# Avielstein/GRASP_LAB_SALP

Measured on AMD Instinct MI355X. Metric: env-steps/sec at 65536 parallel envs, 1/2/4/8 MI355X; % HBM roofline, higher is better.
Workload: dtype f64

## Files before the change

### grasp_lab_salp_amd/csrc/salp_device.h

```cpp
#ifndef SALP_DEVICE_H
#define SALP_DEVICE_H

#include <hip/hip_runtime.h>
#include <stdint.h>

#include "../../include/salp.h"
#include "salp_math.h"
#include "salp_philox.h"
#include "salp_random.h"

#pragma clang fp contract(off)

static_assert(SALP_FMA, "libsalp.so is built in the product arithmetic mode (salp_math.h)");

#define SD static __device__ __forceinline__
#define SD_MEMBER __device__ __forceinline__
#define SD_HOST_DEV static __host__ __device__ __forceinline__

namespace salp {

constexpr double DT = 0.01;
constexpr double PI = 3.141592653589793;
constexpr double COS_GAMMA = 0x1.6a09e667f3bcdp-1;
constexpr double SIN_GAMMA = 0x1.6a09e667f3bccp-1;
// ... 69 lines not shown
    if (d != 0.0 && fabs(d) * 2.0 == fabs(ulp) && e != 0.0) r = ((e > 0) == (d > 0)) ? nb : r;
    return r;
}

struct Rot { double r[3][3]; };
SD Rot rot_sc(double sp, double cp, double st, double ct, double ss, double cs) {
    double a00 = cs * ct, a01 = -ss, a02 = cs * st;
    double a10 = ss * ct, a11 = cs, a12 = ss * st;
    double a20 = -st, a22 = ct;
    Rot R;
    R.r[0][0] = a00; R.r[0][1] = sm_fma(a02, sp, a01 * cp); R.r[0][2] = sm_fma(a02, cp, a01 * -sp);
    R.r[1][0] = a10; R.r[1][1] = sm_fma(a12, sp, a11 * cp); R.r[1][2] = sm_fma(a12, cp, a11 * -sp);
    R.r[2][0] = a20; R.r[2][1] = a22 * sp;                   R.r[2][2] = a22 * cp;
    return R;
}
SD Rot rot_zyx(double phi, double theta, double psi) {
    double sp, cp, st, ct, ss, cs;
    sm_sincos(phi, &sp, &cp);
    sm_sincos(theta, &st, &ct);
    sm_sincos(psi, &ss, &cs);
    return rot_sc(sp, cp, st, ct, ss, cs);
}
SD void world_frame(double e0, double e1, double e2, double v0, double v1, double v2, double* o, SmPoly K) {
    double sp, cp, st, ct, ss, cs;
    sm_sincos_rp2(e0, e1, &sp, &cp, &st, &ct, K);
    sm_sincos_yaw_p(e2, &ss, &cs, K);
    sm_world_frame(sp, cp, st, ct, ss, cs, v0, v1, v2, o);
}
SD void rot_body_xy(const Rot& R, double d0, double d1, double* b0, double* b1) {
    *b0 = sm_fma(R.r[1][0], d1, R.r[0][0] * d0);
    *b1 = sm_fma(R.r[1][1], d1, R.r[0][1] * d0);
}

SD double r32(double x, bool f) { return f ? (double)(float)x : x; }
SD double sel(bool f, double c) { return f ? (double)(float)c : c; }
// ... 319 lines not shown
    SF(SALP_F_POS0) = h.q0; SF(SALP_F_POS1) = h.q1; SF(SALP_F_POS2) = h.q2;
    SF(SALP_F_ANG0) = h.g0; SF(SALP_F_ANG1) = h.g1; SF(SALP_F_ANG2) = h.g2;
    SF(SALP_F_LENGTH) = h.L; SF(SALP_F_WIDTH) = h.W; SF(SALP_F_VOLUME) = h.V;
    SF(SALP_F_PREV_VOLUME) = h.pV; SF(SALP_F_COM) = h.com; SF(SALP_F_COM_RATE) = h.comr;
    SF(SALP_F_COM_ACC) = h.coma;
    SF(SALP_F_PREV_I0) = h.pI0; SF(SALP_F_PREV_I1) = h.pI1; SF(SALP_F_PREV_I2) = h.pI2;
    SF(SALP_F_GEOM32) = h.g32 ? 1.0 : 0.0; SF(SALP_F_PVOL32) = h.pv32 ? 1.0 : 0.0;
    SF(SALP_F_CYCLE_TIME) = h.ct; SF(SALP_F_TIME) = h.time;
    SF(SALP_F_REFILL_TIME) = h.refill; SF(SALP_F_JET_TIME) = h.jet; SF(SALP_F_COAST_TIME) = h.coast;
    SF(SALP_F_CONTRACTION) = h.c; SF(SALP_F_CONTRACT_RATE) = h.cr; SF(SALP_F_RELEASE_RATE) = h.rr;
    SF(SALP_F_TURN_TIME) = h.turn;
    SF(SALP_F_PHASE) = (double)h.phase;
    SF(SALP_F_CONTR32) = h.c32 ? 1.0 : 0.0;
}

SD void nozzle_direction(double angle1, double angle2, double* d) {
    const double cg = COS_GAMMA, sg = SIN_GAMMA;
    double s1, c1, s2, c2;
    sm_sincos(angle1, &s1, &c1);
    sm_sincos(angle2, &s2, &c2);
    double n00 = cg * c2, n10 = s2, n20 = sg * c2;
    double n02 = -sg, n12 = 0.0, n22 = cg;
    double c00 = -n20, c02 = -n22;
    double c10 = sm_fma(c1, n10, s1 * n00), c12 = sm_fma(c1, n12, s1 * n02);
    double c20 = sm_fma(-s1, n10, c1 * n00), c22 = sm_fma(-s1, n12, c1 * n02);
    d[0] = sm_fma(c02, sg, c00 * cg);
    d[1] = sm_fma(c12, sg, c10 * cg);
    d[2] = sm_fma(c22, sg, c20 * cg);
}
SD void cycle_bounds(Hot& h) {
    h.mx = pymax(h.refill, h.turn);
    h.b1 = h.mx + h.jet;
    h.b2 = h.b1 + h.coast;
}

// ... 208 lines not shown
        ng.m = k32[C32_M]; ng.I0 = k32[C32_I0]; ng.I1 = k32[C32_I1];
        ng.kc0 = k32[C32_KC0]; ng.kc1 = k32[C32_KC1]; ng.ra0 = k32[C32_RA0]; ng.ra1 = k32[C32_RA1];
        ng.dimx = k32[C32_DIMX]; ng.dimy = k32[C32_DIMY];
    }
    h.V = V;
    double comr = div_dt(com - h.com);
    h.coma = div_dt(comr - h.comr);
    h.com = com;
    h.comr = comr;
    jet_rates(P, V, h.pV, wm, f, h.pv32, ng);
    geo_recips(ng);
    h.geo = ng;
    return false;
}

SD void nozzle_ik(double yaw, bool yaw32, double* an1_out, double* an2_out) {
    double sy, cy;
    if (yaw32) {
        float s, c;
        sm_np_sincosf((float)yaw, &s, &c);
        sy = s; cy = c;
    } else {
        sm_sincos(yaw, &sy, &cy);
    }
    double t1 = -sy, t2 = cy;
    double val2 = 2.0 * t2 - 1.0;
    if (val2 < -1.0) val2 = -1.0;
    if (val2 > 1.0) val2 = 1.0;
    double an2 = sm_acos(val2), an1;
    if (an2 <= -PI) an2 += 2 * PI;
    else if (an2 > PI) an2 -= 2 * PI;
    if (an2 == 0.0) {
        an1 = 0.0;
    } else {
        double s2, c2;
        sm_sincos(an2, &s2, &c2);
        double a = 0.5 * (c2 - 1.0);
        double b = sqrt(2.0) * s2 / 2.0;
        double val1 = t1 / sqrt(a * a + b * b);
        if (val1 < -1.0) val1 = -1.0;
        if (val1 > 1.0) val1 = 1.0;
        an1 = sm_asin(val1) - sm_atan2(b, a);
    }
    if (an1 <= -PI) an1 += 2 * PI;
    else if (an1 > PI) an1 -= 2 * PI;
    *an1_out = an1;
    *an2_out = an2;
}
template <class ST>
SD void nozzle_solve(ST S, const Params& P, int64_t i, double yaw, bool yaw32) {
    SF(SALP_F_PREV_YAW) = SF(SALP_F_YAW);
    SF(SALP_F_YAW) = yaw;
    SF(SALP_F_PREV_ANGLE1) = SF(SALP_F_ANGLE1);
    SF(SALP_F_PREV_ANGLE2) = SF(SALP_F_ANGLE2);
    double an1, an2;
    nozzle_ik(yaw, yaw32, &an1, &an2);
    SF(SALP_F_ANGLE1) = an1;
    SF(SALP_F_ANGLE2) = an2;
}

SD int predict_cycle_ticks(const Params& P, float a0, float a1, float a2, double* ang1, double* ang2) {
    const float r0 = a0 * 0.06f, r1 = a1 * 10.0f, r2 = a2 * (float)(PI / 2);
    double an1, an2;
    nozzle_ik((double)r2, true, &an1, &an2);
    const double turn = fabs(an1 - *ang1) / P.angle_speed + fabs(an2 - *ang2) / P.angle_speed;
    *ang1 = an1;
    *ang2 = an2;
    const double c = (double)r0, sq = (double)sqf(r0);
    const double refill = REFILL_C0 * sq + REFILL_C1 * c + REFILL_C2;
    const double jet = PROPUL_C0 * sq + PROPUL_C1 * c + PROPUL_C2;
    const double total = pymax(refill, turn) + jet + (double)r1;
// ... 22 lines not shown
    } else {
        sr_coef_means(&k);
    }
    SF(SALP_F_CD) = k.cd; SF(SALP_F_DFR) = k.dfr; SF(SALP_F_DTR) = k.dtr;
#pragma unroll
    for (int j = 0; j < 3; ++j) {
        SF(SALP_F_AMF0 + j) = k.amf[j]; SF(SALP_F_AMRF0 + j) = k.amrf[j];
        SF(SALP_F_AMT0 + j) = k.amt[j]; SF(SALP_F_AMRT0 + j) = k.amrt[j];
    }
    h.rnd.cd = k.cd; h.rnd.dfr = k.dfr; h.rnd.dtr = k.dtr;
    h.rnd.amf0 = k.amf[0]; h.rnd.amf1 = k.amf[1]; h.rnd.amf2 = k.amf[2];
    h.rnd.amrf0 = k.amrf[0]; h.rnd.amrf1 = k.amrf[1]; h.rnd.amrf2 = k.amrf[2];
    h.rnd.amt0 = k.amt[0]; h.rnd.amt1 = k.amt[1]; h.rnd.amt2 = k.amt[2];
}

template <bool RAND = false, class ST>
SD void set_control(Hot& h, ST S, const Params& P, int64_t i, double contraction, double coast,
                    double a1, double a2, bool c32) {
    set_coefficients<RAND>(h, S, P, i);
    SF(SALP_F_AVGV0) = 0.0; SF(SALP_F_AVGV1) = 0.0; SF(SALP_F_AVGV2) = 0.0;
    SF(SALP_F_AVGW0) = 0.0; SF(SALP_F_AVGW1) = 0.0; SF(SALP_F_AVGW2) = 0.0;
    h.c = contraction;
    h.coast = coast;
    h.c32 = c32;
    h.turn = nozzle_set_angles(S, P, i, a1, a2);
    nozzle_direction(a1, a2, &h.d0);
    SF(SALP_F_CYCLE) = SF(SALP_F_CYCLE) + 1.0;
    h.ct = 0.0;
    const double sq = c32 ? (double)sqf((float)h.c) : h.c * h.c;
    h.refill = REFILL_C0 * sq + REFILL_C1 * h.c + REFILL_C2;
    h.jet = PROPUL_C0 * sq + PROPUL_C1 * h.c + PROPUL_C2;
    h.cr = h.refill > 0 ? h.c / h.refill : 0.0;
    h.rr = h.jet > 0 ? h.c / h.jet : 0.0;
    cycle_bounds(h);
}

template <class ST>
SD void cycle_prologue(const Hot& h, ST S, const Params& P, int64_t i) {
    const double total = h.b2;
    double pq0 = SF(SALP_F_PPOS0), pq1 = SF(SALP_F_PPOS1), pq2 = SF(SALP_F_PPOS2);
    double pg0 = SF(SALP_F_PANG0), pg1 = SF(SALP_F_PANG1), pg2 = SF(SALP_F_PANG2);
    SF(SALP_F_AVGV0) = (h.q0 - pq0) / total; SF(SALP_F_AVGV1) = (h.q1 - pq1) / total;
    SF(SALP_F_AVGV2) = (h.q2 - pq2) / total;
    SF(SALP_F_AVGW0) = (h.g0 - pg0) / total; SF(SALP_F_AVGW1) = (h.g1 - pg1) / total;
    SF(SALP_F_AVGW2) = (h.g2 - pg2) / total;
    SF(SALP_F_PPOS0) = h.q0; SF(SALP_F_PPOS1) = h.q1; SF(SALP_F_PPOS2) = h.q2;
    SF(SALP_F_PANG0) = h.g0; SF(SALP_F_PANG1) = h.g1; SF(SALP_F_PANG2) = h.g2;
    SF(SALP_F_PENDING) = 1.0;
}

template <bool RAND = false, class ST>
SD void begin_step(Hot& h, ST S, const Params& P, int64_t i, float a0, float a1, float a2,
                   Cache32 c32) {
    SF(SALP_F_ACT0) = a0; SF(SALP_F_ACT1) = a1; SF(SALP_F_ACT2) = a2;
    float r0 = a0 * 0.06f, r1 = a1 * 10.0f, r2 = a2 * (float)(PI / 2);
    if (RAND && P.rand_act) {
        const float rr[3] = {r0, r1, r2};
        double ra[3];
        sr_randomize_action(P.seed, h.env_id, (uint64_t)SF(SALP_F_STEP_COUNT), rr, ra);
        nozzle_solve(S, P, i, ra[2], false);
        set_control<RAND>(h, S, P, i, ra[0], ra[1], SF(SALP_F_ANGLE1), SF(SALP_F_ANGLE2), false);
    } else {
        nozzle_solve(S, P, i, (double)r2, true);
        set_control<RAND>(h, S, P, i, (double)r0, (double)r1, SF(SALP_F_ANGLE1), SF(SALP_F_ANGLE2), true);
    }
    fill_cache32(P, h.c, c32);
    cycle_prologue(h, S, P, i);
}

template <class ST>
SD void record_state(const Hot& h, const Params& P, ST S, int64_t i, double* rec,
                     int64_t rs, bool first) {
    auto put = [&](int col, double x) { rec[(int64_t)col * rs] = x; };
    put(SALP_T_STATE, (double)h.phase);
    put(SALP_T_PW0, h.p0); put(SALP_T_PW1, h.p1); put(SALP_T_PW2, h.p2);
    put(SALP_T_V0, h.v0); put(SALP_T_V1, h.v1); put(SALP_T_V2, h.v2);
    put(SALP_T_ACC0, h.a0); put(SALP_T_ACC1, h.a1); put(SALP_T_ACC2, h.a2);
    put(SALP_T_ETA0, h.e0); put(SALP_T_ETA1, h.e1); put(SALP_T_ETA2, h.e2);
    put(SALP_T_W0, h.w0); put(SALP_T_W1, h.w1); put(SALP_T_W2, h.w2);
// ... 16 lines not shown
        for (int k = SALP_T_FIRST_FORCE; k < SALP_TRACE_DIM; ++k) put(k, NAN);
        put(SALP_T_ETAR0, NAN); put(SALP_T_ETAR1, NAN); put(SALP_T_ETAR2, NAN);
        put(SALP_T_NOZZLE_YAW, NAN);
    } else {
        const double yaw = SF(SALP_F_YAW), pyaw = SF(SALP_F_PREV_YAW);
        put(SALP_T_NOZZLE_YAW, h.ct < h.turn ? pyaw + (h.ct / h.turn) * (yaw - pyaw) : yaw);
    }
}

template <class ST>
SD void resume_cycle(Hot& h, ST S, const Params& P, int64_t i) {
    cycle_bounds(h);
    nozzle_direction(SF(SALP_F_ANGLE1), SF(SALP_F_ANGLE2), &h.d0);
}

template <class ST>
SD void observation(const Hot& h, const Rot& R, ST S, const Params& P, int64_t i,
                    float* obs) {
    double tx = SF(SALP_F_TARGET0), ty = SF(SALP_F_TARGET1);
    double b0, b1;
    rot_body_xy(R, tx - h.p0, ty - h.p1, &b0, &b1);
    double heading = sm_atan2(b1, b0);
    obs[0] = (float)b0; obs[1] = (float)b1;
    obs[2] = (float)h.v0; obs[3] = (float)h.v1;
    obs[4] = (float)h.w2; obs[5] = (float)heading;
    const int nob = (int)SF(SALP_F_N_OBST);
#pragma unroll
    for (int k = 0; k < SALP_MAX_OBSTACLES; ++k) {
        if (k >= P.num_obstacles) break;
        if (k < nob) {
            obs[6 + 2 * k] = (float)(SF(SALP_F_OBST0 + 2 * k) - h.p0);
            obs[7 + 2 * k] = (float)(SF(SALP_F_OBST0 + 2 * k + 1) - h.p1);
        } else {
            obs[6 + 2 * k] = 0.0f;
            obs[7 + 2 * k] = 0.0f;
        }
    }
}

struct StepOut {
    double reward;
    bool terminated, truncated, hit;
};

template <bool RAND = false, class ST>
SD StepOut finish_step(Hot& h, ST S, const Params& P, int64_t i, float* obs,
                       double* info) {
    StepOut out;
    const Rot R = rot_zyx(h.e0, h.e1, h.e2);
    double vw[3];
    world_frame(h.e0, h.e1, h.e2, h.v0, h.v1, h.v2, vw, sm_poly());
    const double px = h.p0, py = h.p1;
    double path = SF(SALP_F_PATH_LEN) + np_norm2(px - SF(SALP_F_LAST_PX), py - SF(SALP_F_LAST_PY));
    SF(SALP_F_PATH_LEN) = path;
    SF(SALP_F_LAST_PX) = px; SF(SALP_F_LAST_PY) = py;
    double svel = SF(SALP_F_SUM_VEL) + np_norm2(vw[0], vw[1]);
    SF(SALP_F_SUM_VEL) = svel;
    const double tx = SF(SALP_F_TARGET0), ty = SF(SALP_F_TARGET1);
    const double dx = px - tx, dy = py - ty;
    const double dist = np_norm2(dx, dy);
    double comp[7];
    comp[0] = (-dist + SF(SALP_F_PREV_DIST)) * 100;
    SF(SALP_F_PREV_DIST) = dist;
    double b0, b1;
    rot_body_xy(R, dx, dy, &b0, &b1);
    comp[1] = -0.5 * fabs(sm_atan2(-b1, -b0));
    const float a2 = (float)SF(SALP_F_ACT2);
    const double ep_len = SF(SALP_F_EP_LEN);
    if (ep_len == 0.0) {
        double ch = (double)a2 - SF(SALP_F_PREV_A2);
        comp[2] = -1.0 * (ch * ch);
    } else {
        float ch = a2 - (float)SF(SALP_F_PREV_A2);
        comp[2] = (double)(-(ch * ch));
    }
    comp[3] = -10.0 * fabs(SF(SALP_F_AVGW2));
    comp[4] = -0.1;
    comp[5] = -100.0 * fabs(SF(SALP_F_AVGV1));
    comp[6] = 0.0;
    const int nob = (int)SF(SALP_F_N_OBST);
    double md = 0.0;
#pragma unroll
    for (int k = 0; k < SALP_MAX_OBSTACLES; ++k) {
        if (k >= nob) break;
        double d = np_norm2(px - SF(SALP_F_OBST0 + 2 * k), py - SF(SALP_F_OBST0 + 2 * k + 1));
        if (k == 0 || d < md) md = d;
    }
    if (nob > 0) {
        double danger = 2.0 * P.obstacle_radius;
        if (md < danger) comp[6] = -1.0 * (1.0 - md / danger);
    }
    double reward = comp[0] + comp[1] + comp[2] + comp[3] + comp[4] + comp[5] + comp[6];
    observation(h, R, S, P, i, obs);
    if (RAND && P.rand_obs) sr_randomize_obs(P.seed, h.env_id, (uint64_t)SF(SALP_F_STEP_COUNT), obs);
    bool l32;
    double Lc, Wc;
    body_lw(P, h.phase, h.ct, h.refill, h.mx, h.c, h.cr, h.rr, h.c32, &Lc, &Wc, &l32);
    double thr = l32 ? (double)((float)P.obstacle_radius + (float)Lc / 2.0f)
                     : P.obstacle_radius + Lc / 2;
    bool hit = false;
#pragma unroll
    for (int k = 0; k < SALP_MAX_OBSTACLES; ++k) {
        if (k >= nob) break;
        double d = np_norm2(px - SF(SALP_F_OBST0 + 2 * k), py - SF(SALP_F_OBST0 + 2 * k + 1));
        if (d < thr) hit = true;
    }
    bool done = false, trunc = false;
    if (dist < 0.2) { done = true; reward += 500.0; }
    else if (dist > 5.0) { trunc = true; reward -= 200.0; }
    if (hit) { trunc = true; reward -= 200.0; }
    if (SF(SALP_F_CYCLE) >= (double)P.max_cycles) { trunc = true; reward -= 50.0; }
    const double nlen = ep_len + 1.0;
    SF(SALP_F_EP_LEN) = nlen;
    const double ret = SF(SALP_F_EP_RETURN) + reward;
    SF(SALP_F_EP_RETURN) = ret;
    const double sa0 = SF(SALP_F_SUM_A0) + (double)(float)SF(SALP_F_ACT0);
    const double sa1 = SF(SALP_F_SUM_A1) + (double)(float)SF(SALP_F_ACT1);
    const double sa2 = SF(SALP_F_SUM_ABS_A2) + (double)fabsf(a2);
    SF(SALP_F_SUM_A0) = sa0; SF(SALP_F_SUM_A1) = sa1; SF(SALP_F_SUM_ABS_A2) = sa2;
// ... 16 lines not shown
            info[SALP_INFO_DIRECT_DISTANCE] = dd;
            info[SALP_INFO_PATH_EFFICIENCY] = path > 0 ? dd / path : 0.0;
            info[SALP_INFO_FINAL_DISTANCE] = dist;
            info[SALP_INFO_INITIAL_DISTANCE] = SF(SALP_F_INIT_DIST);
            info[SALP_INFO_AVG_COMPRESSION] = sa0 / nlen;
            info[SALP_INFO_AVG_COAST_TIME] = sa1 / nlen;
            info[SALP_INFO_AVG_NOZZLE_ANGLE] = sa2 / nlen;
            info[SALP_INFO_AVG_VELOCITY] = svel / (nlen + 1.0);
            for (int k = 0; k < 7; ++k) info[SALP_INFO_AVG_R_TRACK + k] = sr[k] / nlen;
        }
    }
    SF(SALP_F_PREV_A2) = (double)a2;
    SF(SALP_F_PENDING) = 0.0;
    if (RAND && P.latency) {
        const double lat = sr_latency(P.seed, h.env_id, (uint64_t)SF(SALP_F_STEP_COUNT));
        set_control<RAND>(h, S, P, i, 0.0, lat, SF(SALP_F_ANGLE1), SF(SALP_F_ANGLE2), false);
    }
    out.reward = reward;
    out.terminated = done;
    out.truncated = trunc;
    out.hit = hit;
    return out;
}

SD int draw_reset(const Params& P, uint64_t env_id, uint64_t episode, float* tgt, float* obst) {
    double u0, u1;
    sp_reset_pair(P.seed, env_id, episode, 0u, &u0, &u1);
    double tx = P.x_min + (P.x_max - P.x_min) * u0, ty = P.y_min + (P.y_max - P.y_min) * u1;
    if (tx < P.x_min) tx = P.x_min;
    if (tx > P.x_max) tx = P.x_max;
    if (ty < P.y_min) ty = P.y_min;
// ... 40 lines not shown
    h.coma = (h.comr - h.comr) / DT;
    h.L = P.L0; h.W = P.W0; h.g32 = false;
    const Core c0 = core(h.L, h.W, false);
    h.V = water_volume(P, c0, false);
    h.pV = h.V; h.pv32 = false;
    refresh_derived(h, P);
    h.pI0 = h.geo.I0; h.pI1 = h.geo.I1; h.pI2 = h.geo.I1;
    if (P.rand_dist) {
        SF(SALP_F_OUF0) = 0.0; SF(SALP_F_OUF1) = 0.0; SF(SALP_F_OUF2) = 0.0;
        SF(SALP_F_OUT0) = 0.0; SF(SALP_F_OUT1) = 0.0; SF(SALP_F_OUT2) = 0.0;
        h.rnd.ouf0 = 0.0; h.rnd.ouf1 = 0.0; h.rnd.out2 = 0.0;
    }
    SF(SALP_F_PENDING) = 0.0;
}

template <class ST>
SD void reset_env(Hot& h, ST S, const Params& P, int64_t i, const float* tgt,
                  const float* obst, int nob, float* obs) {
    SF(SALP_F_TARGET0) = tgt[0]; SF(SALP_F_TARGET1) = tgt[1];
#pragma unroll
    for (int k = 0; k < SALP_MAX_OBSTACLES; ++k) {
        SF(SALP_F_OBST0 + 2 * k) = k < nob ? (double)obst[2 * k] : 0.0;
        SF(SALP_F_OBST0 + 2 * k + 1) = k < nob ? (double)obst[2 * k + 1] : 0.0;
    }
    SF(SALP_F_N_OBST) = nob;
    robot_reset(h, S, P, i);
    const double d0 = h.p0 - (double)tgt[0], d1 = h.p1 - (double)tgt[1];
    const double dist = np_norm2(d0, d1);
    SF(SALP_F_PREV_DIST) = dist;
    SF(SALP_F_PREV_A2) = 0.0;
    SF(SALP_F_ACT0) = 0.0; SF(SALP_F_ACT1) = 0.0; SF(SALP_F_ACT2) = 0.0;
    SF(SALP_F_EP_LEN) = 0.0; SF(SALP_F_EP_RETURN) = 0.0; SF(SALP_F_PATH_LEN) = 0.0;
    SF(SALP_F_LAST_PX) = h.p0; SF(SALP_F_LAST_PY) = h.p1;
    SF(SALP_F_SUM_A0) = 0.0; SF(SALP_F_SUM_A1) = 0.0; SF(SALP_F_SUM_ABS_A2) = 0.0;
    SF(SALP_F_SUM_VEL) = np_norm2(0.0, 0.0);
    SF(SALP_F_INIT_DIST) = dist;
#pragma unroll
    for (int k = 0; k < 7; ++k) SF(SALP_F_SUM_R0 + k) = 0.0;
    SF(SALP_F_EPISODE) = SF(SALP_F_EPISODE) + 1.0;
    SF(SALP_F_PENDING) = 0.0;
    if (obs) {
        Rot R = rot_zyx(h.e0, h.e1, h.e2);
        observation(h, R, S, P, i, obs);
    }
}

template <class ST>
SD void reset_env_philox(Hot& h, ST S, const Params& P, int64_t i, float* obs) {
    float tgt[2], obst[2 * SALP_MAX_OBSTACLES];
    int nob = draw_reset(P, (uint64_t)(P.env_offset + i), (uint64_t)SF(SALP_F_EPISODE), tgt, obst);
    reset_env(h, S, P, i, tgt, obst, nob, obs);
}

template <bool RAND>
SD void load_cold(ColdRegs<RAND>& C, double* S, const Params& P, int64_t i) {
    C.g = S + i;
    C.n = P.n;
    if (!SALP_COLD_BLOCK) {
#pragma unroll
        for (int f = 0; f < SALP_NUM_FIELDS; ++f)
            if (is_cached<RAND>(f)) C.v[f] = S[(size_t)f * (size_t)P.n + (size_t)i];
        return;
    }
    const double2* blk = reinterpret_cast<const double2*>(S + P.cold_off + (size_t)i * COLD_SLOTS);
    double v[kLayout.n_cold + 1];
#pragma unroll
// ... 129 lines not shown
```

### grasp_lab_salp_amd/csrc/salp_kernels.hip

```cpp
#include <hip/hip_runtime.h>

#include <cmath>
#include <cstdio>
#include <cstdlib>
#include <cstring>
#include <string>

#include "salp_device.h"
#include "salp_pair.h"
#include "salp_tanh.h"

using salp::Hot;
using salp::Params;

#define SF(f) salp::sref(S, P, i, (f))

namespace {

constexpr int kBlock = 256;
constexpr int kMaxTicksPerCycle = 1 << 16;
constexpr int64_t kSortMinEnvs = 1024;

static_assert(kBlock == salp::LANES, "LDS cache stride is the workgroup size");

// ... 386 lines not shown
    static constexpr bool kDefer = false;
    static constexpr bool kL2 = false;
    __device__ __forceinline__ const float* l2() const { return nullptr; }
    __device__ __forceinline__ void start_rep() {}
    __device__ __forceinline__ void boot(const float*, int, float, int64_t) {}
    __device__ __forceinline__ void value(const float*, int, int64_t) {}
    __device__ __forceinline__ void publish() {}
};

#ifndef SALP_COLLECT_REP_MIN
#define SALP_COLLECT_REP_MIN 4
#endif

__device__ __forceinline__ float clamp_box(float a, float lo, float hi) { return a < lo ? lo : (a > hi ? hi : a); }

template <bool RAND, bool POL, class ST, class VS = ValuesInPlace>
__device__ __forceinline__ void rollout_boundary(Hot& h, ST S, const Params& P, int64_t i,
                                                 uint64_t env_id, bool& pending, bool& active,
                                                 int64_t& steps, int64_t max_steps,
                                                 const SalpRolloutBuffers& B, double* reward_sum,
                                                 const SalpPolicyRollout& R, salp::Cache32 c32, VS vs = VS()) {
    float o[SALP_OBS_DIM_MAX];
    bool have_o = false;
    float ep_start = 0.0f;
    for (int rep = 0; rep < 4; ++rep) {
        const bool fin = active && pending && !(h.ct < h.b2);
        vs.start_rep();
        if (fin) {
            SF(SALP_F_STEP_COUNT) = SF(SALP_F_STEP_COUNT) + 1.0;
            salp::StepOut r = salp::finish_step<RAND>(h, S, P, i, o, nullptr);
            bool reset = r.terminated || r.truncated;
            if (POL) {
                const size_t row = (size_t)steps * (size_t)P.n + (size_t)i;
                float rew = (float)r.reward;
                bool bad = false;
                if (R.diverged_obs_abs > 0.0) {
                    bad = !(fabs(r.reward) <= R.diverged_reward_abs);
                    for (int k = 0; k < P.obs_dim; ++k) bad = bad || !(fabsf(o[k]) <= (float)R.diverged_obs_abs);
                }
                if (bad) {
                    rew = 0.0f;
                    atomicAdd((unsigned long long*)R.diverged, 1ull);
                } else if (r.truncated && !r.terminated) {
                    if (VS::kDefer) {
                        vs.boot(o, P.obs_dim, rew, (int64_t)steps);
// ... 17 lines not shown
                const size_t slot = (size_t)(steps % B.capacity);
                const size_t row = slot * (size_t)P.n + (size_t)i;
                if (B.obs)
                    for (int k = 0; k < P.obs_dim; ++k) B.obs[row * P.obs_dim + k] = o[k];
                if (B.actions) {
                    B.actions[row * 3 + 0] = (float)SF(SALP_F_ACT0);
                    B.actions[row * 3 + 1] = (float)SF(SALP_F_ACT1);
                    B.actions[row * 3 + 2] = (float)SF(SALP_F_ACT2);
                }
                if (B.rewards) B.rewards[row] = (float)r.reward;
                if (B.dones) B.dones[row] = (uint8_t)((r.terminated ? 1 : 0) | (r.truncated ? 2 : 0));
            }
            if (reward_sum) reward_sum[i] += r.reward;
            ++steps;
            pending = false;
            if (reset) salp::reset_env_philox(h, S, P, i, (POL || B.obs_before) ? o : nullptr);
            have_o = true;
            if (max_steps > 0 && steps >= max_steps) {
                active = false;
                if (POL)
                    for (int k = 0; k < P.obs_dim; ++k) R.last_obs[(size_t)i * P.obs_dim + k] = o[k];
            }
        }
        const bool beg = active && !pending;
        if (beg) {
            if (POL && !have_o) {
                for (int k = 0; k < P.obs_dim; ++k) o[k] = R.last_obs[(size_t)i * P.obs_dim + k];
                have_o = true;
            } else if (B.obs_before && !have_o) {
                const salp::Rot Rt = salp::rot_zyx(h.e0, h.e1, h.e2);
                salp::observation(h, Rt, S, P, i, o);
                have_o = true;
            }
            if (POL && VS::kDefer) vs.value(o, P.obs_dim, (int64_t)steps);
        }
        vs.publish();
        if (beg) {
            float a[3];
            if (POL) {
                if (!fin) ep_start = R.episode_start[i];
                float raw[3], v, lp;
                policy_act<VS::kL2>(R, P.obs_dim, o, env_id, (uint64_t)SF(SALP_F_STEP_COUNT), raw,
                                    VS::kDefer ? nullptr : &v, &lp, vs.l2());
                const size_t row = (size_t)steps * (size_t)P.n + (size_t)i;
                for (int k = 0; k < P.obs_dim; ++k) R.obs[row * P.obs_dim + k] = o[k];
                R.actions[row * 3 + 0] = raw[0];
                R.actions[row * 3 + 1] = raw[1];
                R.actions[row * 3 + 2] = raw[2];
                if (!VS::kDefer) R.values[row] = v;
                R.log_probs[row] = lp;
                R.episode_starts[row] = ep_start;
                a[0] = clamp_box(raw[0], 0.0f, 1.0f);
                a[1] = clamp_box(raw[1], 0.0f, 1.0f);
                a[2] = clamp_box(raw[2], -1.0f, 1.0f);
            } else {
                if (B.obs_before && B.capacity > 0) {
                    const size_t row = (size_t)(steps % B.capacity) * (size_t)P.n + (size_t)i;
                    for (int k = 0; k < P.obs_dim; ++k) B.obs_before[row * P.obs_dim + k] = o[k];
                }
                sp_action(P.seed, env_id, (uint64_t)SF(SALP_F_STEP_COUNT), a);
            }
            salp::begin_step<RAND>(h, S, P, i, a[0], a[1], a[2], c32);
            pending = true;
        }
        if (POL && SALP_COLLECT_REP_MIN > 1) {
            const bool again = active && pending && !(h.ct < h.b2);
            if (__popcll(__ballot(again)) < SALP_COLLECT_REP_MIN) break;
        }
        if (VS::kDefer) {
            if (!__any(fin || beg)) break;
        } else if (!fin && !beg) {
            break;
        }
    }
}

struct RolloutArgs {
    double* S;
    Params P;
// ... 51 lines not shown
            pos += half;
        } else {
            w = lo;
        }
    }
    return base + pos;
}

__device__ __forceinline__ bool unsteady(const Hot& h, const Params& P, bool active) {
    return active && h.ct < h.b2 && !salp::next_tick_steady(h, P);
}

template <bool RAND, bool POL>
__device__ __forceinline__ bool lane_boundary(const RolloutArgs& a, salp::SpillSlot sp, int64_t i, bool& pending,
                                              bool& active, int64_t& steps, double* c32p) {
    const uint64_t env_id = (uint64_t)(a.P.env_offset + i);
    salp::ColdRegs<RAND> C;
    salp::load_cold<RAND>(C, a.S, a.P, i);
    Hot hb;
    salp::unspill<RAND>(hb, sp, a.P, env_id);
    rollout_boundary<RAND, POL>(hb, &C, a.P, i, env_id, pending, active, steps, a.max_steps, a.B,
                                a.reward_sum, a.R, salp::Cache32{c32p});
    salp::store_cold<RAND>(C, a.S, a.P, i);
    salp::spill<RAND>(hb, sp);
    return unsteady(hb, a.P, active);
}
template <bool RAND, bool POL>
__device__ __noinline__ bool lane_boundary_call(const RolloutArgs* a, double* spp, int64_t i, bool* pending,
                                                bool* active, int64_t* steps, double* c32p) {
    return lane_boundary<RAND, POL>(*a, salp::SpillSlot{spp}, i, *pending, *active, *steps, c32p);
}

#ifndef SALP_ROLLOUT_PROF
#define SALP_ROLLOUT_PROF 0
#endif
enum { RP_BOUNDARY, RP_FULL, RP_STEADY, RP_SETTLED, RP_BARRIER, RP_RESEAT, RP_N };
__device__ unsigned long long g_roll_prof[2][RP_N];
struct RollProf {
    unsigned long long cyc[RP_N] = {}, its[RP_N] = {};
    unsigned long long t = 0;
// ... 24 lines not shown
    const uint32_t lo = __builtin_amdgcn_readfirstlane((uint32_t)kernarg);
    const uint32_t hi = __builtin_amdgcn_readfirstlane((uint32_t)(kernarg >> 32));
    return args_at((KernargWords)(((uint64_t)hi << 32) | lo));
}
__device__ __forceinline__ uint32_t tick_flags(const Hot& h, const Params& P, bool active) {
    return (uint32_t)((h.ct < h.b2 ? TK_TICKING : 0) | (unsteady(h, P, active) ? TK_UNSTEADY : 0));
}
#if SALP_ROLLOUT_PROF
#define ROLL_PROF_PARAM , RollProf& prof
#define ROLL_PROF_ARG , prof
#else
#define ROLL_PROF_PARAM
#define ROLL_PROF_ARG
#endif
template <bool RAND>
[[clang::not_tail_called]] __device__ __noinline__ uint32_t wave_ticks(uint64_t kernarg, LdsDouble* spp,
                                                                       LdsDouble* c32p, int64_t i,
                                                                       uint32_t active ROLL_PROF_PARAM) {
#if !SALP_ROLLOUT_PROF
    RollProf prof;
#endif
    const salp::SpillSlot sp{(double*)spp};
    const salp::Cache32 c32{(double*)c32p};
    const RolloutArgs A = args_of(kernarg);
    const int32_t chunk = A.chunk, steady_q8 = A.steady_q8;
    Hot h;
    salp::unspill<RAND>(h, sp, A.P, (uint64_t)(A.P.env_offset + i));
    if (!active) h.b2 = -INFINITY;
    prof.lap(RP_RESEAT);
    const Params PV = salp::pin_params(A.P);
    int32_t k = 0;
// ... 1008 lines not shown
    out[13 * n + i] = cy;
    sm_sincos_rp2(x[i], y[i], &s0, &c0, &s1, &c1, sm_poly());
    out[14 * n + i] = s0;
    out[15 * n + i] = c0;
    out[16 * n + i] = s1;
    out[17 * n + i] = c1;
    sm_sincos_yaw_p(x[i] + y[i], &sz, &cz, sm_poly());
    sm_world_frame(s0, c0, s1, c1, sz, cz, y[i], x[i], 1.0, wf);
    out[18 * n + i] = wf[0];
    out[19 * n + i] = wf[1];
    out[20 * n + i] = wf[2];
    out[21 * n + i] = sm_atan(x[i]);
    out[22 * n + i] = sm_atan_ref(x[i]);
}

const char* const kFieldNames[SALP_NUM_FIELDS] = {
    "v0", "v1", "v2", "w0", "w1", "w2", "acc0", "acc1", "acc2", "alpha0", "alpha1", "alpha2",
    "eta0", "eta1", "eta2", "pw0", "pw1", "pw2", "pos0", "pos1", "pos2", "ang0", "ang1", "ang2",
    "ppos0", "ppos1", "ppos2", "pang0", "pang1", "pang2", "avgv0", "avgv1", "avgv2",
    "avgw0", "avgw1", "avgw2",
    "length", "width", "volume", "prev_volume", "com", "com_rate", "com_acc",
    "prev_I0", "prev_I1", "prev_I2", "geom32", "pvol32",
    "cycle_time", "time", "refill_time", "jet_time", "coast_time", "contraction",
    "contract_rate", "release_rate", "phase", "cycle", "contr32",
    "angle1", "angle2", "prev_angle1", "prev_angle2", "yaw", "prev_yaw", "turn_time",
    "target0", "target1", "obst0", "obst1", "obst2", "obst3", "obst4", "obst5", "obst6", "obst7",
    "n_obst", "prev_dist", "prev_a2",
    "ep_len", "ep_return", "path_len", "last_px", "last_py", "sum_a0", "sum_a1", "sum_abs_a2",
    "sum_vel", "init_dist", "sum_r0", "sum_r1", "sum_r2", "sum_r3", "sum_r4", "sum_r5", "sum_r6",
    "act0", "act1", "act2", "pending", "step_count", "episode",
// ... 482 lines not shown
}

int salp_set_lockstep_order(SalpEnv* h, int mode) {
    if (!h) return fail(nullptr, SALP_EINVAL, "salp_set_lockstep_order: null handle");
    if (mode < -1 || mode > 1) return fail(h, SALP_EINVAL, "salp_set_lockstep_order: mode must be -1, 0 or 1");
    h->order_mode = mode;
    return SALP_OK;
}

#if SALP_ROLLOUT_PROF
int salp_debug_rollout_prof(unsigned long long* out) {
    if (hipMemcpyFromSymbol(out, HIP_SYMBOL(g_roll_prof), sizeof(g_roll_prof)) != hipSuccess) return -1;
    static const unsigned long long zero[2][RP_N] = {};
    return hipMemcpyToSymbol(HIP_SYMBOL(g_roll_prof), zero, sizeof zero) == hipSuccess ? 0 : -1;
}
#endif

#if SALP_PAIR_PROF
int salp_debug_pair_prof(unsigned long long* out) {
    if (hipMemcpyFromSymbol(out, HIP_SYMBOL(g_pair_prof), sizeof(g_pair_prof)) != hipSuccess) return -1;
    static const unsigned long long zero[2][PP_N] = {};
    return hipMemcpyToSymbol(HIP_SYMBOL(g_pair_prof), zero, sizeof zero) == hipSuccess ? 0 : -1;
}
#endif

int salp_pair_timeouts(SalpEnv* h, uint64_t* count_out, void* stream) {
    if (!h || !count_out) return fail(h, SALP_EINVAL, "salp_pair_timeouts: null argument");
    unsigned int c = 0;
    const hipStream_t s = (hipStream_t)stream;
    hipError_t e = hipMemcpyFromSymbolAsync(&c, HIP_SYMBOL(g_pair_timeouts), sizeof c, 0, hipMemcpyDeviceToHost, s);
// ... 266 lines not shown
```

Measured before the change: 74.74 million.

## Outline boundary-step trig into noinline callees and reuse cached angles

Measured after the change: 75.42 million, median of 6. About the same (+0.9%).

```diff
diff --git a/grasp_lab_salp_amd/csrc/salp_device.h b/grasp_lab_salp_amd/csrc/salp_device.h
--- a/grasp_lab_salp_amd/csrc/salp_device.h
+++ b/grasp_lab_salp_amd/csrc/salp_device.h
@@ -107,11 +107,39 @@
     R.r[2][0] = a20; R.r[2][1] = a22 * sp;                   R.r[2][2] = a22 * cp;
     return R;
 }
+#define SD_CALLEE [[clang::not_tail_called]] static __device__ __noinline__
+struct SinCos { double s, c; };
+SD_CALLEE double atan2_called(double y, double x) { return sm_atan2(y, x); }
+SD_CALLEE SinCos sincos_called(double x) {
+    SinCos r;
+    sm_sincos(x, &r.s, &r.c);
+    return r;
+}
+template <bool LEAN>
+SD double bd_atan2(double y, double x) {
+    if constexpr (LEAN) return atan2_called(y, x);
+    else return sm_atan2(y, x);
+}
+template <bool LEAN>
+SD double bd_asin(double x) { return bd_atan2<LEAN>(x, sqrt((1.0 - x) * (1.0 + x))); }
+template <bool LEAN>
+SD double bd_acos(double x) { return bd_atan2<LEAN>(sqrt((1.0 - x) * (1.0 + x)), x); }
+template <bool LEAN>
+SD void bd_sincos(double x, double* s, double* c) {
+    if constexpr (LEAN) {
+        const SinCos r = sincos_called(x);
+        *s = r.s;
+        *c = r.c;
+    } else {
+        sm_sincos(x, s, c);
+    }
+}
+template <bool LEAN = false>
 SD Rot rot_zyx(double phi, double theta, double psi) {
     double sp, cp, st, ct, ss, cs;
-    sm_sincos(phi, &sp, &cp);
-    sm_sincos(theta, &st, &ct);
-    sm_sincos(psi, &ss, &cs);
+    bd_sincos<LEAN>(phi, &sp, &cp);
+    bd_sincos<LEAN>(theta, &st, &ct);
+    bd_sincos<LEAN>(psi, &ss, &cs);
     return rot_sc(sp, cp, st, ct, ss, cs);
 }
 SD void world_frame(double e0, double e1, double e2, double v0, double v1, double v2, double* o, SmPoly K) {
@@ -461,11 +489,12 @@
     SF(SALP_F_CONTR32) = h.c32 ? 1.0 : 0.0;
 }
 
+template <bool LEAN = false>
 SD void nozzle_direction(double angle1, double angle2, double* d) {
     const double cg = COS_GAMMA, sg = SIN_GAMMA;
     double s1, c1, s2, c2;
-    sm_sincos(angle1, &s1, &c1);
-    sm_sincos(angle2, &s2, &c2);
+    bd_sincos<LEAN>(angle1, &s1, &c1);
+    bd_sincos<LEAN>(angle2, &s2, &c2);
     double n00 = cg * c2, n10 = s2, n20 = sg * c2;
     double n02 = -sg, n12 = 0.0, n22 = cg;
     double c00 = -n20, c02 = -n22;
@@ -704,6 +733,7 @@
     return false;
 }
 
+template <bool LEAN = false>
 SD void nozzle_ik(double yaw, bool yaw32, double* an1_out, double* an2_out) {
     double sy, cy;
     if (yaw32) {
@@ -711,40 +741,40 @@
         sm_np_sincosf((float)yaw, &s, &c);
         sy = s; cy = c;
     } else {
-        sm_sincos(yaw, &sy, &cy);
+        bd_sincos<LEAN>(yaw, &sy, &cy);
     }
     double t1 = -sy, t2 = cy;
     double val2 = 2.0 * t2 - 1.0;
     if (val2 < -1.0) val2 = -1.0;
     if (val2 > 1.0) val2 = 1.0;
-    double an2 = sm_acos(val2), an1;
+    double an2 = bd_acos<LEAN>(val2), an1;
     if (an2 <= -PI) an2 += 2 * PI;
     else if (an2 > PI) an2 -= 2 * PI;
     if (an2 == 0.0) {
         an1 = 0.0;
     } else {
         double s2, c2;
-        sm_sincos(an2, &s2, &c2);
+        bd_sincos<LEAN>(an2, &s2, &c2);
         double a = 0.5 * (c2 - 1.0);
         double b = sqrt(2.0) * s2 / 2.0;
         double val1 = t1 / sqrt(a * a + b * b);
         if (val1 < -1.0) val1 = -1.0;
         if (val1 > 1.0) val1 = 1.0;
-        an1 = sm_asin(val1) - sm_atan2(b, a);
+        an1 = bd_asin<LEAN>(val1) - bd_atan2<LEAN>(b, a);
     }
     if (an1 <= -PI) an1 += 2 * PI;
     else if (an1 > PI) an1 -= 2 * PI;
     *an1_out = an1;
     *an2_out = an2;
 }
-template <class ST>
+template <bool LEAN = false, class ST>
 SD void nozzle_solve(ST S, const Params& P, int64_t i, double yaw, bool yaw32) {
     SF(SALP_F_PREV_YAW) = SF(SALP_F_YAW);
     SF(SALP_F_YAW) = yaw;
     SF(SALP_F_PREV_ANGLE1) = SF(SALP_F_ANGLE1);
     SF(SALP_F_PREV_ANGLE2) = SF(SALP_F_ANGLE2);
     double an1, an2;
-    nozzle_ik(yaw, yaw32, &an1, &an2);
+    nozzle_ik<LEAN>(yaw, yaw32, &an1, &an2);
     SF(SALP_F_ANGLE1) = an1;
     SF(SALP_F_ANGLE2) = an2;
 }
@@ -797,7 +827,7 @@
     h.rnd.amt0 = k.amt[0]; h.rnd.amt1 = k.amt[1]; h.rnd.amt2 = k.amt[2];
 }
 
-template <bool RAND = false, class ST>
+template <bool RAND = false, bool LEAN = false, class ST>
 SD void set_control(Hot& h, ST S, const Params& P, int64_t i, double contraction, double coast,
                     double a1, double a2, bool c32) {
     set_coefficients<RAND>(h, S, P, i);
@@ -807,7 +837,7 @@
     h.coast = coast;
     h.c32 = c32;
     h.turn = nozzle_set_angles(S, P, i, a1, a2);
-    nozzle_direction(a1, a2, &h.d0);
+    nozzle_direction<LEAN>(a1, a2, &h.d0);
     SF(SALP_F_CYCLE) = SF(SALP_F_CYCLE) + 1.0;
     h.ct = 0.0;
     const double sq = c32 ? (double)sqf((float)h.c) : h.c * h.c;
@@ -832,7 +862,7 @@
     SF(SALP_F_PENDING) = 1.0;
 }
 
-template <bool RAND = false, class ST>
+template <bool RAND = false, bool LEAN = false, class ST>
 SD void begin_step(Hot& h, ST S, const Params& P, int64_t i, float a0, float a1, float a2,
                    Cache32 c32) {
     SF(SALP_F_ACT0) = a0; SF(SALP_F_ACT1) = a1; SF(SALP_F_ACT2) = a2;
@@ -841,11 +871,11 @@
         const float rr[3] = {r0, r1, r2};
         double ra[3];
         sr_randomize_action(P.seed, h.env_id, (uint64_t)SF(SALP_F_STEP_COUNT), rr, ra);
-        nozzle_solve(S, P, i, ra[2], false);
-        set_control<RAND>(h, S, P, i, ra[0], ra[1], SF(SALP_F_ANGLE1), SF(SALP_F_ANGLE2), false);
+        nozzle_solve<LEAN>(S, P, i, ra[2], false);
+        set_control<RAND, LEAN>(h, S, P, i, ra[0], ra[1], SF(SALP_F_ANGLE1), SF(SALP_F_ANGLE2), false);
     } else {
-        nozzle_solve(S, P, i, (double)r2, true);
-        set_control<RAND>(h, S, P, i, (double)r0, (double)r1, SF(SALP_F_ANGLE1), SF(SALP_F_ANGLE2), true);
+        nozzle_solve<LEAN>(S, P, i, (double)r2, true);
+        set_control<RAND, LEAN>(h, S, P, i, (double)r0, (double)r1, SF(SALP_F_ANGLE1), SF(SALP_F_ANGLE2), true);
     }
     fill_cache32(P, h.c, c32);
     cycle_prologue(h, S, P, i);
@@ -892,13 +922,13 @@
     nozzle_direction(SF(SALP_F_ANGLE1), SF(SALP_F_ANGLE2), &h.d0);
 }
 
-template <class ST>
-SD void observation(const Hot& h, const Rot& R, ST S, const Params& P, int64_t i,
-                    float* obs) {
+template <bool LEAN = false, class ST>
+SD double observation(const Hot& h, const Rot& R, ST S, const Params& P, int64_t i,
+                      float* obs) {
     double tx = SF(SALP_F_TARGET0), ty = SF(SALP_F_TARGET1);
     double b0, b1;
     rot_body_xy(R, tx - h.p0, ty - h.p1, &b0, &b1);
-    double heading = sm_atan2(b1, b0);
+    double heading = bd_atan2<LEAN>(b1, b0);
     obs[0] = (float)b0; obs[1] = (float)b1;
     obs[2] = (float)h.v0; obs[3] = (float)h.v1;
     obs[4] = (float)h.w2; obs[5] = (float)heading;
@@ -914,6 +944,7 @@
             obs[7 + 2 * k] = 0.0f;
         }
     }
+    return heading;
 }
 
 struct StepOut {
@@ -921,13 +952,19 @@
     bool terminated, truncated, hit;
 };
 
-template <bool RAND = false, class ST>
+template <bool RAND = false, bool LEAN = false, class ST>
 SD StepOut finish_step(Hot& h, ST S, const Params& P, int64_t i, float* obs,
                        double* info) {
     StepOut out;
-    const Rot R = rot_zyx(h.e0, h.e1, h.e2);
+    const Rot R = rot_zyx<LEAN>(h.e0, h.e1, h.e2);
     double vw[3];
-    world_frame(h.e0, h.e1, h.e2, h.v0, h.v1, h.v2, vw, sm_poly());
+    if (LEAN) {
+        double ss, cs;
+        sm_sincos_yaw_p(h.e2, &ss, &cs, sm_poly());
+        sm_world_frame(h.sp, h.cp, h.st, h.cth, ss, cs, h.v0, h.v1, h.v2, vw);
+    } else {
+        world_frame(h.e0, h.e1, h.e2, h.v0, h.v1, h.v2, vw, sm_poly());
+    }
     const double px = h.p0, py = h.p1;
     double path = SF(SALP_F_PATH_LEN) + np_norm2(px - SF(SALP_F_LAST_PX), py - SF(SALP_F_LAST_PY));
     SF(SALP_F_PATH_LEN) = path;
@@ -942,7 +979,15 @@
     SF(SALP_F_PREV_DIST) = dist;
     double b0, b1;
     rot_body_xy(R, dx, dy, &b0, &b1);
-    comp[1] = -0.5 * fabs(sm_atan2(-b1, -b0));
+    if (LEAN) {
+        const double heading = observation<LEAN>(h, R, S, P, i, obs);
+        const bool zeros = dx == 0.0 || dy == 0.0 || b0 == 0.0 || b1 == 0.0;
+        double rh = heading;
+        if (__any(zeros)) rh = bd_atan2<LEAN>(-b1, -b0);
+        comp[1] = -0.5 * fabs(rh);
+    } else {
+        comp[1] = -0.5 * fabs(sm_atan2(-b1, -b0));
+    }
     const float a2 = (float)SF(SALP_F_ACT2);
     const double ep_len = SF(SALP_F_EP_LEN);
     if (ep_len == 0.0) {
@@ -958,10 +1003,12 @@
     comp[6] = 0.0;
     const int nob = (int)SF(SALP_F_N_OBST);
     double md = 0.0;
+    double od[SALP_MAX_OBSTACLES];
 #pragma unroll
     for (int k = 0; k < SALP_MAX_OBSTACLES; ++k) {
         if (k >= nob) break;
         double d = np_norm2(px - SF(SALP_F_OBST0 + 2 * k), py - SF(SALP_F_OBST0 + 2 * k + 1));
+        if (LEAN) od[k] = d;
         if (k == 0 || d < md) md = d;
     }
     if (nob > 0) {
@@ -969,7 +1016,7 @@
         if (md < danger) comp[6] = -1.0 * (1.0 - md / danger);
     }
     double reward = comp[0] + comp[1] + comp[2] + comp[3] + comp[4] + comp[5] + comp[6];
-    observation(h, R, S, P, i, obs);
+    if (!LEAN) observation(h, R, S, P, i, obs);
     if (RAND && P.rand_obs) sr_randomize_obs(P.seed, h.env_id, (uint64_t)SF(SALP_F_STEP_COUNT), obs);
     bool l32;
     double Lc, Wc;
@@ -980,7 +1027,7 @@
 #pragma unroll
     for (int k = 0; k < SALP_MAX_OBSTACLES; ++k) {
         if (k >= nob) break;
-        double d = np_norm2(px - SF(SALP_F_OBST0 + 2 * k), py - SF(SALP_F_OBST0 + 2 * k + 1));
+        double d = LEAN ? od[k] : np_norm2(px - SF(SALP_F_OBST0 + 2 * k), py - SF(SALP_F_OBST0 + 2 * k + 1));
         if (d < thr) hit = true;
     }
     bool done = false, trunc = false;
@@ -1027,7 +1074,7 @@
     SF(SALP_F_PENDING) = 0.0;
     if (RAND && P.latency) {
         const double lat = sr_latency(P.seed, h.env_id, (uint64_t)SF(SALP_F_STEP_COUNT));
-        set_control<RAND>(h, S, P, i, 0.0, lat, SF(SALP_F_ANGLE1), SF(SALP_F_ANGLE2), false);
+        set_control<RAND, LEAN>(h, S, P, i, 0.0, lat, SF(SALP_F_ANGLE1), SF(SALP_F_ANGLE2), false);
     }
     out.reward = reward;
     out.terminated = done;
@@ -1098,7 +1145,7 @@
     SF(SALP_F_PENDING) = 0.0;
 }
 
-template <class ST>
+template <bool LEAN = false, class ST>
 SD void reset_env(Hot& h, ST S, const Params& P, int64_t i, const float* tgt,
                   const float* obst, int nob, float* obs) {
     SF(SALP_F_TARGET0) = tgt[0]; SF(SALP_F_TARGET1) = tgt[1];
@@ -1125,15 +1172,15 @@
     SF(SALP_F_PENDING) = 0.0;
     if (obs) {
         Rot R = rot_zyx(h.e0, h.e1, h.e2);
-        observation(h, R, S, P, i, obs);
-    }
-}
-
-template <class ST>
+        observation<LEAN>(h, R, S, P, i, obs);
+    }
+}
+
+template <bool LEAN = false, class ST>
 SD void reset_env_philox(Hot& h, ST S, const Params& P, int64_t i, float* obs) {
     float tgt[2], obst[2 * SALP_MAX_OBSTACLES];
     int nob = draw_reset(P, (uint64_t)(P.env_offset + i), (uint64_t)SF(SALP_F_EPISODE), tgt, obst);
-    reset_env(h, S, P, i, tgt, obst, nob, obs);
+    reset_env<LEAN>(h, S, P, i, tgt, obst, nob, obs);
 }
 
 template <bool RAND>
diff --git a/grasp_lab_salp_amd/csrc/salp_kernels.hip b/grasp_lab_salp_amd/csrc/salp_kernels.hip
--- a/grasp_lab_salp_amd/csrc/salp_kernels.hip
+++ b/grasp_lab_salp_amd/csrc/salp_kernels.hip
@@ -424,12 +424,49 @@
 
 __device__ __forceinline__ float clamp_box(float a, float lo, float hi) { return a < lo ? lo : (a > hi ? hi : a); }
 
-template <bool RAND, bool POL, class ST, class VS = ValuesInPlace>
+#ifndef SALP_ROLLOUT_PROF
+#define SALP_ROLLOUT_PROF 0
+#endif
+#if SALP_ROLLOUT_PROF
+enum { BP_LOAD, BP_FINISH, BP_RESET, BP_BEGIN, BP_STORE, BP_N };
+__device__ unsigned long long g_bound_prof[3][BP_N];
+struct BoundProf {
+    unsigned long long cyc[BP_N] = {}, waves[BP_N] = {}, lanes[BP_N] = {};
+    unsigned long long t = 0;
+    __device__ __forceinline__ void start() { t = __builtin_amdgcn_s_memtime(); }
+    __device__ __forceinline__ void lap(int part, bool mine) {
+        const unsigned long long now = __builtin_amdgcn_s_memtime();
+        const unsigned long long n = (unsigned long long)__popcll(__ballot(mine));
+        cyc[part] += now - t;
+        waves[part] += n ? 1ull : 0ull;
+        lanes[part] += n;
+        t = now;
+    }
+    __device__ __forceinline__ void flush() {
+        if ((threadIdx.x & 63) == 0)
+            for (int k = 0; k < BP_N; ++k) {
+                atomicAdd(&g_bound_prof[0][k], cyc[k]);
+                atomicAdd(&g_bound_prof[1][k], waves[k]);
+                atomicAdd(&g_bound_prof[2][k], lanes[k]);
+            }
+    }
+};
+#define BOUND_PROF_PARAM , BoundProf* bp = nullptr
+#define BOUND_PROF_ARG , ValuesInPlace(), &bp
+#define BOUND_LAP(part, mine) \
+    if (bp) bp->lap(part, mine)
+#else
+#define BOUND_PROF_PARAM
+#define BOUND_PROF_ARG
+#define BOUND_LAP(part, mine)
+#endif
+template <bool RAND, bool POL, bool LEAN = false, class ST, class VS = ValuesInPlace>
 __device__ __forceinline__ void rollout_boundary(Hot& h, ST S, const Params& P, int64_t i,
                                                  uint64_t env_id, bool& pending, bool& active,
                                                  int64_t& steps, int64_t max_steps,
                                                  const SalpRolloutBuffers& B, double* reward_sum,
-                                                 const SalpPolicyRollout& R, salp::Cache32 c32, VS vs = VS()) {
+                                                 const SalpPolicyRollout& R, salp::Cache32 c32,
+                                                 VS vs = VS() BOUND_PROF_PARAM) {
     float o[SALP_OBS_DIM_MAX];
     bool have_o = false;
     float ep_start = 0.0f;
@@ -438,7 +475,7 @@
         vs.start_rep();
         if (fin) {
             SF(SALP_F_STEP_COUNT) = SF(SALP_F_STEP_COUNT) + 1.0;
-            salp::StepOut r = salp::finish_step<RAND>(h, S, P, i, o, nullptr);
+            salp::StepOut r = salp::finish_step<RAND, LEAN>(h, S, P, i, o, nullptr);
             bool reset = r.terminated || r.truncated;
             if (POL) {
                 const size_t row = (size_t)steps * (size_t)P.n + (size_t)i;
@@ -486,7 +523,9 @@
             if (reward_sum) reward_sum[i] += r.reward;
             ++steps;
             pending = false;
-            if (reset) salp::reset_env_philox(h, S, P, i, (POL || B.obs_before) ? o : nullptr);
+            BOUND_LAP(BP_FINISH, true);
+            if (reset) salp::reset_env_philox<LEAN>(h, S, P, i, (POL || B.obs_before) ? o : nullptr);
+            BOUND_LAP(BP_RESET, reset);
             have_o = true;
             if (max_steps > 0 && steps >= max_steps) {
                 active = false;
@@ -500,8 +539,8 @@
                 for (int k = 0; k < P.obs_dim; ++k) o[k] = R.last_obs[(size_t)i * P.obs_dim + k];
                 have_o = true;
             } else if (B.obs_before && !have_o) {
-                const salp::Rot Rt = salp::rot_zyx(h.e0, h.e1, h.e2);
-                salp::observation(h, Rt, S, P, i, o);
+                const salp::Rot Rt = salp::rot_zyx<LEAN>(h.e0, h.e1, h.e2);
+                salp::observation<LEAN>(h, Rt, S, P, i, o);
                 have_o = true;
             }
             if (POL && VS::kDefer) vs.value(o, P.obs_dim, (int64_t)steps);
@@ -532,9 +571,10 @@
                 }
                 sp_action(P.seed, env_id, (uint64_t)SF(SALP_F_STEP_COUNT), a);
             }
-            salp::begin_step<RAND>(h, S, P, i, a[0], a[1], a[2], c32);
+            salp::begin_step<RAND, LEAN>(h, S, P, i, a[0], a[1], a[2], c32);
             pending = true;
         }
+        BOUND_LAP(BP_BEGIN, beg);
         if (POL && SALP_COLLECT_REP_MIN > 1) {
             const bool again = active && pending && !(h.ct < h.b2);
             if (__popcll(__ballot(again)) < SALP_COLLECT_REP_MIN) break;
@@ -616,16 +656,28 @@
 template <bool RAND, bool POL>
 __device__ __forceinline__ bool lane_boundary(const RolloutArgs& a, salp::SpillSlot sp, int64_t i, bool& pending,
                                               bool& active, int64_t& steps, double* c32p) {
+#if SALP_ROLLOUT_PROF
+    BoundProf bp;
+    bp.start();
+#endif
     const uint64_t env_id = (uint64_t)(a.P.env_offset + i);
     salp::ColdRegs<RAND> C;
     salp::load_cold<RAND>(C, a.S, a.P, i);
     Hot hb;
     salp::unspill<RAND>(hb, sp, a.P, env_id);
-    rollout_boundary<RAND, POL>(hb, &C, a.P, i, env_id, pending, active, steps, a.max_steps, a.B,
-                                a.reward_sum, a.R, salp::Cache32{c32p});
+#if SALP_ROLLOUT_PROF
+    bp.lap(BP_LOAD, true);
+#endif
+    rollout_boundary<RAND, POL, !RAND>(hb, &C, a.P, i, env_id, pending, active, steps, a.max_steps, a.B,
+                                       a.reward_sum, a.R, salp::Cache32{c32p} BOUND_PROF_ARG);
     salp::store_cold<RAND>(C, a.S, a.P, i);
     salp::spill<RAND>(hb, sp);
-    return unsteady(hb, a.P, active);
+    const bool uns = unsteady(hb, a.P, active);
+#if SALP_ROLLOUT_PROF
+    bp.lap(BP_STORE, true);
+    bp.flush();
+#endif
+    return uns;
 }
 template <bool RAND, bool POL>
 __device__ __noinline__ bool lane_boundary_call(const RolloutArgs* a, double* spp, int64_t i, bool* pending,
@@ -680,7 +732,7 @@
 #define ROLL_PROF_ARG
 #endif
 template <bool RAND>
-[[clang::not_tail_called]] __device__ __noinline__ uint32_t wave_ticks(uint64_t kernarg, LdsDouble* spp,
+[[clang::not_tail_called]] __attribute__((aligned(256))) __device__ __noinline__ uint32_t wave_ticks(uint64_t kernarg, LdsDouble* spp,
                                                                        LdsDouble* c32p, int64_t i,
                                                                        uint32_t active ROLL_PROF_PARAM) {
 #if !SALP_ROLLOUT_PROF
@@ -1719,6 +1771,13 @@
     out[22 * n + i] = sm_atan_ref(x[i]);
 }
 
+__global__ __attribute__((used)) void k_boundary_callee_probe(const double* x, double* out) {
+    const salp::SinCos sc = salp::sincos_called(x[0]);
+    out[0] = salp::atan2_called(x[0], x[1]);
+    out[1] = sc.s;
+    out[2] = sc.c;
+}
+
 const char* const kFieldNames[SALP_NUM_FIELDS] = {
     "v0", "v1", "v2", "w0", "w1", "w2", "acc0", "acc1", "acc2", "alpha0", "alpha1", "alpha2",
     "eta0", "eta1", "eta2", "pw0", "pw1", "pw2", "pos0", "pos1", "pos2", "ang0", "ang1", "ang2",
@@ -2231,6 +2290,11 @@
     static const unsigned long long zero[2][RP_N] = {};
     return hipMemcpyToSymbol(HIP_SYMBOL(g_roll_prof), zero, sizeof zero) == hipSuccess ? 0 : -1;
 }
+int salp_debug_boundary_prof(unsigned long long* out) {
+    if (hipMemcpyFromSymbol(out, HIP_SYMBOL(g_bound_prof), sizeof(g_bound_prof)) != hipSuccess) return -1;
+    static const unsigned long long zero[3][BP_N] = {};
+    return hipMemcpyToSymbol(HIP_SYMBOL(g_bound_prof), zero, sizeof zero) == hipSuccess ? 0 : -1;
+}
 #endif
 
 #if SALP_PAIR_PROF
```
